# adjust/pg_cryogen

Hardware: AMD Instinct MI355X
Metric: lz4_decompress_uncompressed_GBps (higher is better)
Workload: dtype u8

## Files before the change

pg_cryogen_amd/csrc/lz4_index_pair.hip:

```cpp
#include "lz_common.h"

namespace cryo {
namespace {

constexpr uint32_t kIdxDist = 2;
constexpr uint32_t kIdxLanes = 64, kIdxRing = 512;
constexpr uint32_t kIdxLpw = 8u;
constexpr uint32_t kIdxChunk = kIdxLpw * 16u;
constexpr uint32_t kIdxWpl = kIdxLanes / kIdxLpw;
constexpr uint32_t kIdxGroups = kIdxLanes / (2u * kIdxWpl);
constexpr uint32_t kIdxLine = 16u;
constexpr uint32_t kIdxStride = kIdxRing + 16u;

constexpr uint32_t kPairTrash = kIdxLanes * kIdxStride;
constexpr uint32_t kPairPos = kPairTrash + kIdxLanes * 16u;
constexpr uint32_t kPairPosStride = (2u * kIdxLine + 8u) * 2u;
constexpr uint32_t kPairMbPos = kPairPos + kIdxLanes * kPairPosStride;
constexpr uint32_t kPairMbFilled = kPairMbPos + kIdxLanes * 4u;
constexpr uint32_t kPairLds = kPairMbFilled + kIdxLanes * 4u;
static_assert(4u * kPairLds <= 163840u, "four pairs per compute unit");

constexpr uint32_t kPairStarve = 65536u;
constexpr uint32_t kPairIdle = 65536u;

__device__ inline uint32_t pair_bperm(uint32_t v, uint32_t src_lane)
{
    return (uint32_t)__builtin_amdgcn_ds_bpermute((int)(src_lane << 2), (int)v);
}
__device__ inline uint32_t mb_load(const uint32_t *p) { return __hip_atomic_load(p, __ATOMIC_RELAXED, __HIP_MEMORY_SCOPE_WORKGROUP); }
__device__ inline void mb_store(uint32_t *p, uint32_t v) { __hip_atomic_store(p, v, __ATOMIC_RELAXED, __HIP_MEMORY_SCOPE_WORKGROUP); }

#ifndef CRYO_IDX_PAIR_WG
#define CRYO_IDX_PAIR_WG 1
#endif
#ifndef CRYO_IDX_PAIR_PRIO
#define CRYO_IDX_PAIR_PRIO 1
#endif

}

template <uint32_t PAIRS, bool PRIO>
__global__ void __launch_bounds__(128 * PAIRS)
k_lz4_idx_pair(const uint8_t *__restrict__ src_base, const uint64_t *__restrict__ src_off,
               const uint32_t *__restrict__ src_size, const uint64_t n_blocks, uint16_t *__restrict__ tbl,
               const uint32_t cap, uint2 *__restrict__ seg, uint16_t *__restrict__ dummy_base)
{
    __shared__ __attribute__((aligned(16))) uint8_t s_mem[PAIRS * kPairLds];
    const uint32_t wave = uni(threadIdx.x >> 6), lane = threadIdx.x & 63u;
    const bool feeder = wave >= PAIRS;
    const uint32_t pair = feeder ? wave - PAIRS : wave;
    uint8_t *const s_ring = s_mem + pair * kPairLds;
    uint32_t *const mb_pos = reinterpret_cast<uint32_t *>(s_ring + kPairMbPos);
    uint32_t *const mb_filled = reinterpret_cast<uint32_t *>(s_ring + kPairMbFilled);

    const uint64_t blk = ((uint64_t)blockIdx.x * PAIRS + pair) * kIdxLanes + lane;
    const bool owner = blk < n_blocks;
// ... 8 lines not shown
    const bool start_done = !owner || vend == delta;
    if (!feeder) {
        mb_pos[lane] = delta | (start_done ? 0x80000000u : 0u);
        mb_filled[lane] = 0u;
    }
    __syncthreads();

    if (feeder) {
        uint32_t requested = 0, filled = 0;
        uint32_t outA = 0, outB = 0;
        uint32_t lastp = delta;
        const uint32_t piece16 = (lane & (kIdxLpw - 1u)) * 16u;
        const uint32_t wil = lane / kIdxLpw;
#define PAIR_SRC(q) const uint64_t saoff##q = ((uint64_t)pair_bperm((uint32_t)(aoff >> 32), kIdxWpl * q + wil) << 32) | pair_bperm((uint32_t)aoff, kIdxWpl * q + wil); \
                    const uint32_t svend##q = pair_bperm(vend, kIdxWpl * q + wil);
        PAIR_SRC(0) PAIR_SRC(1) PAIR_SRC(2) PAIR_SRC(3)
        PAIR_SRC(4) PAIR_SRC(5) PAIR_SRC(6) PAIR_SRC(7)
#undef PAIR_SRC
        typedef uint32_t u32x4 __attribute__((ext_vector_type(4)));
        const uint32_t mytrash = kPairTrash + lane * 16u;
#define PAIR_SLOT(n) u32x4 fd##n = {0, 0, 0, 0}, fe##n = fd##n; uint32_t fa##n = mytrash, fb##n = fa##n;
        PAIR_SLOT(0) PAIR_SLOT(1) PAIR_SLOT(2) PAIR_SLOT(3)
        PAIR_SLOT(4) PAIR_SLOT(5) PAIR_SLOT(6) PAIR_SLOT(7)
#undef PAIR_SLOT
        uint32_t moved = 0;
        bool alldone = false;
        auto turn = [&](const uint32_t j, u32x4 &fd, u32x4 &fe, uint32_t &fa, uint32_t &fb, uint32_t &out128,
                        const uint64_t soff, const uint32_t sve, const uint64_t soff2, const uint32_t sve2) __attribute__((always_inline)) {
            const uint32_t grp = j % kIdxGroups;
            const bool myturn = lane / (2u * kIdxWpl) == grp;
            asm volatile("s_waitcnt vmcnt(%0)" ::"n"(8 * kIdxDist - 2) : "memory");
            *reinterpret_cast<u32x4 *>(s_ring + fa) = fd;
            *reinterpret_cast<u32x4 *>(s_ring + fb) = fe;
            asm volatile("" ::: "memory");
            {
                const uint32_t got = myturn ? out128 : 0u;
                filled += got;
                out128 -= got;
            }
            const uint32_t pm = mb_load(mb_pos + lane);
            const uint32_t p = pm & 0x7fffffffu;
            const bool pdone = (pm >> 31) != 0u;
            moved |= p ^ lastp;
            lastp = p;
            const bool jump = !pdone & (p >= requested) & (p < vend);
            requested = jump ? p & ~(kIdxChunk - 1u) : requested;
            filled = jump ? requested : filled;
            outA = jump ? 0u : outA;
            outB = jump ? 0u : outB;
            mb_store(mb_filled + lane, filled);
            const bool want = myturn & !pdone & (requested < vend) & (p + (kIdxRing - kIdxChunk) >= requested);
            const uint32_t wi = want ? 1u : 0u;
            const uint32_t msg = requested | wi;
            requested += wi * kIdxChunk;
            out128 |= wi * kIdxChunk;
            moved |= wi;
            const uint32_t s1 = 2u * kIdxWpl * grp + wil, s2 = s1 + kIdxWpl;
            const uint32_t m1 = pair_bperm(msg, s1), m2 = pair_bperm(msg, s2);
            const uint32_t o1 = (m1 & ~1u) + piece16, o2 = (m2 & ~1u) + piece16;
            const bool p1 = (m1 & 1u) != 0u, p2 = (m2 & 1u) != 0u;
            fa = p1 ? s1 * kIdxStride + (o1 & (kIdxRing - 1u)) : mytrash;
            fb = p2 ? s2 * kIdxStride + (o2 & (kIdxRing - 1u)) : mytrash;
            const uint8_t *g1 = src_base + (soff + ((p1 & (o1 < sve)) ? o1 : 0u));
            const uint8_t *g2 = src_base + (soff2 + ((p2 & (o2 < sve2)) ? o2 : 0u));
            asm volatile("global_load_dwordx4 %0, %1, off" : "+v"(fd) : "v"(g1));
            asm volatile("global_load_dwordx4 %0, %1, off" : "+v"(fe) : "v"(g2));
// ... 5 lines not shown
#ifdef CRYO_IDX_PROF
        const unsigned long long t_f0 = __builtin_amdgcn_s_memtime();
        uint32_t prof_rounds = 0;
#endif
        if (!wave_all(start_done)) {
            do {
                PAIR_ROUND(0, 1, 2, 3, outA)
                PAIR_ROUND(4, 5, 6, 7, outB)
#ifdef CRYO_IDX_PROF
                prof_rounds += 2u;
#endif
                idle = wave_any(moved != 0u) ? 0u : idle + 2u;
                moved = 0;
            } while (!alldone && idle < kPairIdle);
        }
#undef PAIR_ROUND
#undef PAIR_TURN
#ifdef CRYO_IDX_PROF
        if ((blockIdx.x & 255u) == 0u && lane == 0u)
            printf("[pair] feeder %u.%u: %u rounds, %llu ticks\n", blockIdx.x, pair, prof_rounds, __builtin_amdgcn_s_memtime() - t_f0);
#endif
        asm volatile("s_waitcnt vmcnt(0)" : "+v"(fd0), "+v"(fe0), "+v"(fd1), "+v"(fe1), "+v"(fd2), "+v"(fe2), "+v"(fd3), "+v"(fe3),
                                            "+v"(fd4), "+v"(fe4), "+v"(fd5), "+v"(fe5), "+v"(fd6), "+v"(fe6), "+v"(fd7), "+v"(fe7) : : "memory");
    } else {
        if (PRIO) __builtin_amdgcn_s_setprio(1);
        uint16_t *const row = tbl + blk * cap;
        uint16_t *const dummy = dummy_base + lane * 16u;
        const uint32_t kcap = cap;
        const uint32_t rb = lane * kIdxStride;
        uint32_t pos = delta, state = 0, acc = 0, tm = 0;
        uint32_t k = 0, ls = 0;
        uint32_t starved = 0;
        uint16_t *const pbuf = reinterpret_cast<uint16_t *>(s_ring + kPairPos + lane * kPairPosStride);
        uint16_t *const ptrash = pbuf + 2u * kIdxLine;
        bool done = start_done;
#ifdef CRYO_IDX_PROF
        uint32_t prof_dry = 0, prof_live = 0, prof_turns = 0;
        const unsigned long long t_w0 = __builtin_amdgcn_s_memtime();
#endif
        auto turn = [&]() __attribute__((always_inline)) {
            const uint32_t filled = mb_load(mb_filled + lane);
            asm volatile("" ::: "memory");
            const uint32_t w0 = *reinterpret_cast<const uint32_t *>(s_ring + rb + (pos & (kIdxRing - 4u)));
            const uint32_t w1 = *reinterpret_cast<const uint32_t *>(s_ring + rb + ((pos + 4u) & (kIdxRing - 4u)));
            const uint32_t w2 = *reinterpret_cast<const uint32_t *>(s_ring + rb + ((pos + 8u) & (kIdxRing - 4u)));
            const bool live = !done & (pos < vend);
            const bool canread = (pos + 8u <= filled) | (filled >= vend);
            const uint32_t x = __builtin_amdgcn_alignbyte(w1, w0, pos & 3u);
            const bool go = live & canread;
            starved = (live & !canread) ? starved + 1u : 0u;
#ifdef CRYO_IDX_PROF
            prof_dry += (live & !canread) ? 1u : 0u;
            prof_live += live ? 1u : 0u;
#endif
            const uint32_t ll = (x >> 4) & 15u, e1 = (x >> 8) & 255u, tmn = x & 15u;
            const bool l15 = ll == 15u;
            const uint32_t q2 = pos + 3u + ll + (l15 ? e1 + 1u : 0u);
            const bool tok = go & (state == 0u);
            const bool rare = tok & ((l15 & (e1 == 255u)) | (q2 > vend));
            const bool plain = tok & !rare;
            const uint32_t nx = ~x;
            const uint32_t n = nx ? (uint32_t)__builtin_ctz(nx) >> 3 : 4u;
            const bool extb = go & (state == 2u);
            *(tok ? pbuf + (k & (2u * kIdxLine - 1u)) : ptrash) = (uint16_t)(pos - delta);
            k += tok ? 1u : 0u;
            tm = tok ? tmn : tm;
            const uint32_t st_tok = tmn == 15u ? 2u : 0u;
            uint32_t npos = plain ? q2 : pos, nstate = plain ? st_tok : state;
            {
                const bool dbl = plain & !l15 & (tmn != 15u) & (ll <= 2u) & (q2 < vend) & (k < kcap);
                const uint32_t x1 = __builtin_amdgcn_alignbyte(w2, w1, pos & 3u);
                const unsigned long long xx = ((unsigned long long)x1 << 32) | x;
                const uint32_t y = (uint32_t)(xx >> (8u * (3u + ll)));
                const uint32_t llb = (y >> 4) & 15u, e1b = (y >> 8) & 255u, tmb = y & 15u;
                const bool l15b = llb == 15u;
                const uint32_t q2b = q2 + 3u + llb + (l15b ? e1b + 1u : 0u);
                const bool rec2 = dbl & !(l15b & (e1b == 255u));
                *(rec2 ? pbuf + (k & (2u * kIdxLine - 1u)) : ptrash) = (uint16_t)(q2 - delta);
                k += rec2 ? 1u : 0u;
                tm = rec2 ? tmb : tm;
                const bool last2 = rec2 & (q2b > vend);
                const bool adv2 = rec2 & !last2;
                npos = adv2 ? q2b : npos;
                nstate = adv2 ? (tmb == 15u ? 2u : 0u) : nstate;
                done = done | last2;
            }
            npos = extb ? pos + (n == 4u ? 4u : n + 1u) : npos;
            nstate = extb ? (n == 4u ? 2u : 0u) : nstate;
            done = done | !live | (k >= kcap) | (starved >= kPairStarve);
            pos = npos;
            state = nstate;
            {
                const bool longm = extb & (n == 4u) & !done;
                if (__builtin_expect(wave_any(longm), 0)) {
                    const uint32_t a0 = pos & ~3u;
                    uint32_t m = 0;
                    bool run = longm;
#pragma unroll
                    for (uint32_t kq = 0; kq < 7u; kq++) {
                        const uint32_t dq = *reinterpret_cast<const uint32_t *>(s_ring + rb + ((a0 + 4u * kq) & (kIdxRing - 4u)));
                        run = run & (dq == 0xffffffffu) & (a0 + 4u * kq + 4u <= filled);
                        m += run ? 1u : 0u;
                    }
                    const uint32_t far = a0 + 4u * m;
                    pos = (longm & (far > pos)) ? far : pos;
                }
            }
            const bool slow = rare | (!done & (state == 1u));
            if (__builtin_expect(wave_any(slow), 0)) {
                if (rare) {
                    if (l15 && e1 == 255u) { state = 1u; acc = 15u + 255u; pos += 2u; }
                    else done = true;
                } else if (slow && pos < vend && live && canread) {
                    if (n == 4u) { acc += 1020u; pos += 4u; if (acc >= vend) done = true; }
                    else {
                        acc += 255u * n + ((x >> (8u * n)) & 255u);
                        const uint32_t q = pos + n + 1u + acc;
                        if (acc >= vend || q + 2u > vend) done = true;
                        else { pos = q + 2u; state = tm == 15u ? 2u : 0u; }
                    }
                }
            }
            mb_store(mb_pos + lane, pos | (done ? 0x80000000u : 0u));
        };
#define PAIR_LINE_COPY(ps_, pd_)                                                                 \
        {                                                                                        \
            const uint4 v0_ = *reinterpret_cast<const uint4 *>(ps_);                             \
            const uint4 v1_ = *reinterpret_cast<const uint4 *>((ps_) + 8);                       \
            store16_out<false>(reinterpret_cast<uint8_t *>(pd_), v0_);                           \
            store16_out<false>(reinterpret_cast<uint8_t *>((pd_) + 8), v1_);                     \
        }
#define PAIR_PUT()                                                                               \
        {                                                                                        \
            const bool st_ = ls < k / kIdxLine;                                                  \
            const uint16_t *ps_ = pbuf + (ls & 1u) * kIdxLine;                                   \
            uint16_t *pd_ = st_ ? row + ls * kIdxLine : dummy;                                   \
            PAIR_LINE_COPY(ps_, pd_)                                                             \
            if (st_) ls++;                                                                       \
        }
        if (wave_any(!done)) {
            do {
                PAIR_PUT()
                turn(); turn(); turn(); turn();
#ifdef CRYO_IDX_PROF
                prof_turns += 4u;
#endif
            } while (wave_any(!done));
        }
#ifdef CRYO_IDX_PROF
        if ((blockIdx.x & 255u) == 0u && lane < 2u)
            printf("[pair] walker %u.%u lane %u: %u turns, live %u, dry %u, %llu ticks, k %u\n", blockIdx.x, pair, lane, prof_turns, prof_live, prof_dry,
                   __builtin_amdgcn_s_memtime() - t_w0, k);
#endif
        if (owner) {
            PAIR_PUT()
            PAIR_PUT()
            if ((k & (kIdxLine - 1u)) != 0u && ls == k / kIdxLine) {
                const uint16_t *ps_ = pbuf + (ls & 1u) * kIdxLine;
                uint16_t *pd_ = row + ls * kIdxLine;
                PAIR_LINE_COPY(ps_, pd_)
            }
            seg[blk] = make_uint2(0u, k);
        }
#undef PAIR_PUT
#undef PAIR_LINE_COPY
        if (PRIO) __builtin_amdgcn_s_setprio(0);
    }
    __syncthreads();
}

hipError_t launch_lz4_index_pair(hipStream_t s, const uint8_t *d_src, const uint64_t *d_src_off, const uint32_t *d_src_size,
                                 uint64_t n_blocks, uint32_t block_size, void *d_workspace, const Lz4IndexLayout &L)
{
    (void)block_size;
    if (n_blocks == 0) return hipSuccess;
    if (L.logS != 0u) return hipErrorInvalidValue;
    constexpr uint32_t kWg = CRYO_IDX_PAIR_WG;
    const uint64_t grid = (n_blocks + kIdxLanes * kWg - 1) / (kIdxLanes * kWg);
    if (grid > 0x7fffffffull) return hipErrorInvalidValue;
    uint8_t *ws = static_cast<uint8_t *>(d_workspace);
    hipLaunchKernelGGL((k_lz4_idx_pair<kWg, CRYO_IDX_PAIR_PRIO != 0>), dim3((uint32_t)grid), dim3(128u * kWg), 0, s, d_src, d_src_off,
                       d_src_size, n_blocks, reinterpret_cast<uint16_t *>(ws), L.cap, reinterpret_cast<uint2 *>(ws + L.seg_off),
                       reinterpret_cast<uint16_t *>(ws + L.dummy_off));
    return hipGetLastError();
}
// ... 25 lines not shown
```

pg_cryogen_amd/csrc/lz4_copy.h:

```cpp
#ifndef CRYO_LZ4_COPY_H
#define CRYO_LZ4_COPY_H

#include "lz_common.h"

namespace cryo {
namespace {

#define LDS_FENCE() asm volatile("" ::: "memory")

template <uint32_t R, uint32_t TMAX>
struct CopyLds {
    static constexpr uint32_t kBmW = TMAX / 32;
    static constexpr uint32_t kNc = TMAX / 64;
    static constexpr uint32_t kWords = kBmW + kNc;
    uint8_t *ring;
    uint8_t *in;
    uint32_t *mmeta;
    uint32_t *mbm;
};

template <uint32_t R, uint32_t SMASK>
__device__ inline void lane_runs(uint8_t *ring, const uint8_t *sbase, uint32_t rem, uint32_t sv, uint32_t dv, const bool far,
                                 const uint4 xa, const uint4 xb, uint32_t &spill)
{
    uint32_t it = 0;
    bool go = rem >= 16u;
    if (wave_any(go)) {
        do {
            const uint32_t di = dv & (R - 1u);
            if (go) {
                uint4 v = it == 0u ? xa : xb;
                if (!far) __builtin_memcpy(&v, sbase + (sv & SMASK), 16);
                __builtin_memcpy(ring + di, &v, 16);
            }
            if (go && di + 16u > R) spill = di + 16u - R;
            const uint32_t step = go ? 16u : 0u;
            sv += step; dv += step; rem -= step; it += step;
            go = rem >= 16u;
        } while (wave_any(go));
    }
    const bool lap = rem != 0u && it != 0u && !far;
    if (lap) {
        uint4 v;
        __builtin_memcpy(&v, sbase + ((sv + rem - 16u) & SMASK), 16);
        const uint32_t di = (dv + rem - 16u) & (R - 1u);
        __builtin_memcpy(ring + di, &v, 16);
        if (di + 16u > R) spill = di + 16u - R;
        rem = 0u;
    }
    if (rem != 0u) {
        uint4 v = it == 0u ? xa : xb;
        if (!far) __builtin_memcpy(&v, sbase + (sv & SMASK), 16);
        uint32_t di = dv & (R - 1u);
        if (di + rem > R) spill = di + rem - R;
        if (rem & 8u) { __builtin_memcpy(ring + di, &v.x, 8); di += 8u; v.x = v.z; v.y = v.w; }
        if (rem & 4u) { __builtin_memcpy(ring + di, &v.x, 4); di += 4u; v.x = v.y; }
        if (rem & 2u) { const uint16_t h = (uint16_t)v.x; __builtin_memcpy(ring + di, &h, 2); di += 2u; v.x >>= 16; }
        if (rem & 1u) ring[di] = (uint8_t)v.x;
    }
}


template <uint32_t R>
__device__ inline void lane_tail_pieces(uint8_t *ring, uint4 v, const uint32_t rem, uint32_t di, uint32_t &spill)
{
    if (di + rem > R) spill = di + rem - R;
    if (rem & 8u) { __builtin_memcpy(ring + di, &v.x, 8); di += 8u; v.x = v.z; v.y = v.w; }
    if (rem & 4u) { __builtin_memcpy(ring + di, &v.x, 4); di += 4u; v.x = v.y; }
    if (rem & 2u) { const uint16_t h = (uint16_t)v.x; __builtin_memcpy(ring + di, &h, 2); di += 2u; v.x >>= 16; }
    if (rem & 1u) ring[di] = (uint8_t)v.x;
}
template <uint32_t R, uint32_t N, typename T>
__device__ inline void lane_store(uint8_t *ring, const uint32_t dv, const T &v, uint32_t &spill)
{
    const uint32_t di = dv & (R - 1u);
    __builtin_memcpy(ring + di, &v, N);
    if (di + N > R) spill = di + N - R;
}

template <uint32_t R>
__device__ inline void lane_copies_v2(uint8_t *ring, const uint8_t *in, const uint32_t L, const uint32_t lpos, const uint32_t dl,
                                      const uint32_t ML, const uint32_t msrc, const uint32_t dm, const bool isfar,
                                      const uint4 xfa, const uint4 xfb, uint32_t &spill)
{
    uint4 la = make_uint4(0, 0, 0, 0), lc = la, ma = xfa;
    const bool l2 = L > 16u && L <= 32u;
    if (L != 0u) __builtin_memcpy(&la, in + (lpos & kInMask), 16);
    if (l2) __builtin_memcpy(&lc, in + ((lpos + L - 16u) & kInMask), 16);
    if (ML != 0u && !isfar) __builtin_memcpy(&ma, ring + (msrc & (R - 1u)), 16);
    if (L >= 16u) lane_store<R, 16>(ring, dl, la, spill);
    if (l2) lane_store<R, 16>(ring, dl + L - 16u, lc, spill);
    if (ML == 16u || (ML > 16u && isfar)) lane_store<R, 16>(ring, dm, ma, spill);
    if (ML >= 8u && ML < 16u) {
        const uint32_t s = ML - 8u;
        const bool hi = s >= 4u;
        const uint32_t a = hi ? ma.y : ma.x, b = hi ? ma.z : ma.y, c = hi ? ma.w : ma.z;
        const uint2 head = make_uint2(ma.x, ma.y);
        const uint2 tail = make_uint2(__builtin_amdgcn_alignbyte(b, a, s), __builtin_amdgcn_alignbyte(c, b, s));
        lane_store<R, 8>(ring, dm, head, spill);
        lane_store<R, 8>(ring, dm + s, tail, spill);
    }
    if (ML >= 4u && ML < 8u) {
        const uint32_t s = ML - 4u;
        const uint32_t tail = __builtin_amdgcn_alignbyte(ma.y, ma.x, s);
        lane_store<R, 4>(ring, dm, ma.x, spill);
        lane_store<R, 4>(ring, dm + s, tail, spill);
    }
    const bool lshort = L != 0u && L < 16u, mshort = ML != 0u && ML < 4u;
    if (wave_any(lshort | mshort)) {
        if (lshort) lane_tail_pieces<R>(ring, la, L, dl & (R - 1u), spill);
        if (mshort) lane_tail_pieces<R>(ring, ma, ML, dm & (R - 1u), spill);
    }
    if (wave_any(L > 32u)) {
        const uint4 z = make_uint4(0, 0, 0, 0);
        lane_runs<R, kInMask>(ring, in, L > 32u ? L - 16u : 0u, lpos + 16u, dl + 16u, false, z, z, spill);
    }
    if (wave_any(ML > 16u)) {
        const uint32_t done = isfar ? 16u : 0u;
        lane_runs<R, R - 1u>(ring, ring, ML > 16u ? ML - done : 0u, msrc + done, dm + done, isfar, xfb, xfb, spill);
    }
}

template <uint32_t R, uint32_t TMAX, bool NOLIT = false>
__device__ inline void seq_copy(Wave<R> &w, const CopyLds<R, TMAX> &L, const uint32_t nseq, const uint32_t ostart,
                                const uint32_t ll, const uint32_t ml, const uint32_t off, const uint32_t lpos,
                                const uint32_t T, const bool isfar, const uint4 xfa, const uint4 xfb, Stats &st)
{
    static_assert(R - TMAX >= TMAX + 1023u, "an offset must be either in the ring or flushed");
    constexpr uint32_t kBmW = CopyLds<R, TMAX>::kBmW, kNc = CopyLds<R, TMAX>::kNc;
    const uint32_t lane = w.lane;
    const uint32_t op0 = w.op;
    const bool act = lane < nseq;
    st.batches++;
    st.batch_seqs += nseq;

    const uint32_t mrel = ostart + ll;
    const bool indep = act && (isfar || off >= mrel + ml);
    const bool dep = act && !indep;
    const uint32_t mlx = dep ? ml : 0u;
    const uint32_t mend = scan64_incl(mlx);
    const uint32_t mcum = mend - mlx;
    const uint32_t MT = lane_get(mend, 63u);
    const unsigned long long depm = wave_ballot(dep);
    const uint32_t drank = __builtin_amdgcn_mbcnt_hi((uint32_t)(depm >> 32), __builtin_amdgcn_mbcnt_lo((uint32_t)depm, 0u));

    {
    if (lane < kBmW) L.mbm[lane] = 0u;
    LDS_FENCE();
    if (dep) {
        static_assert(TMAX < 2048u, "11 bits");
        L.mmeta[drank] = (mrel - mcum) | (off << 11);
        if (mcum != 0u) atomicOr(&L.mbm[(mcum - 1u) >> 5], 1u << ((mcum - 1u) & 31u));
    }
    LDS_FENCE();
// ... 94 lines not shown
```

pg_cryogen_amd/csrc/lz4_dec2.hip:

```cpp
#include "lz_common.h"
#include "lz4_copy.h"
#include <cstdio>
#include <cstdlib>

namespace cryo {


constexpr uint32_t kSeqWin = 1536;
constexpr uint32_t kT2 = 1536;

template <bool MULTI>
struct IndexRow {
    const uint16_t *base;
    uint2 sd;
    uint32_t cap_s, ext, npieces, pc;
    const uint16_t *t0, *t1, *t2;
    uint32_t len0, len1, len2, n0;

    __device__ inline void find(const uint16_t *&t, uint32_t &len)
    {
        len = 0;
        t = base;
        while (pc < npieces) {
            const uint32_t sg = pc >> 1;
            const uint32_t dx = lane_get(sd.x, sg), dy = lane_get(sd.y, sg);
            const uint32_t l = (pc & 1u) ? dy : (dx & 0xffffu);
            const uint32_t b = sg * cap_s + ((pc & 1u) ? ext + (dx >> 16) : 0u);
            pc++;
            if (l != 0u) { t = base + b; len = l; break; }
        }
    }
    __device__ inline void open(const uint16_t *row, const uint2 *seg, const uint64_t blk, const uint32_t logS, const uint32_t cap_s_,
                                const uint32_t ext_, const uint32_t lane)
    {
        base = row;
        cap_s = cap_s_; ext = ext_;
        npieces = 2u << logS;
        sd = make_uint2(0, 0);
        if (lane < (1u << logS)) sd = seg[(blk << logS) + lane];
        pc = 0; n0 = 0;
        find(t0, len0);
        t1 = t2 = base; len1 = len2 = 0;
        if (MULTI) { find(t1, len1); find(t2, len2); }
    }
    __device__ inline uint32_t avail(const uint32_t k) const
    {
        const uint32_t have = MULTI ? len0 + len1 + len2 : len0, at = n0 + k;
        return at < have ? (have - at < 64u ? have - at : 64u) : 0u;
    }
    __device__ inline uint32_t entry(const uint32_t k, const uint32_t lane) const
    {
        const uint32_t i = n0 + k + lane;
        uint32_t e = 0;
        if (MULTI) {
            const uint16_t *q = i < len0 ? t0 + i : (i < len0 + len1 ? t1 + (i - len0) : t2 + (i - len0 - len1));
            if (i < len0 + len1 + len2) e = *q;
        } else if (i < len0) e = t0[i];
        return e;
    }
    __device__ inline void advance(const uint32_t n)
    {
        n0 += n;
        while (MULTI && len0 != 0u && n0 >= len0) {
            n0 -= len0;
            t0 = t1; len0 = len1;
            t1 = t2; len1 = len2;
            find(t2, len2);
        }
    }
};

__device__ inline uint32_t lane_next(uint32_t v)
{
    return (uint32_t)__builtin_amdgcn_update_dpp(0, (int)v, 0x130 , 0xf, 0xf, false);
}

template <uint32_t R, bool MULTI>
__device__ inline uint32_t lz4_seq_batch(Wave<R> &w, const CopyLds<R, kT2> &L, uint32_t &vp, const uint32_t B,
                                         const uint32_t epos, const uint32_t navail, const IndexRow<MULTI> &ix, uint32_t &epre, Stats &st,
                                         unsigned long long *stop_hist = nullptr)
{
    const uint32_t lane = w.lane;
    const uint32_t vend = w.vend;
    if (vend < 32u || B < 32u || navail == 0u) return 0;
    const uint32_t vsafe = vend - 16u;
    if (vp + 64u > vsafe || w.op + 64u > B) return 0;
    stamp(st, 7);
    while (w.in_hi < vend && w.in_hi < vp + kSeqWin) w.refill_deferred();
    LDS_FENCE();
    uint2 mir = make_uint2(0, 0);
    if (lane < 2u) mir = *reinterpret_cast<const uint2 *>(L.in + lane * 8u);
    else if (lane < 4u) mir = *reinterpret_cast<const uint2 *>(L.ring + (lane - 2u) * 8u);
    stamp(st, 0);
    const uint32_t pos = vp + ((epos + w.delta - vp) & 0xffffu);
    const bool cand = lane < navail && pos + 8u <= vp + kSeqWin;
    const uint32_t rp = cand ? pos : vp;
    const uint32_t t = L.in[rp & kInMask];
    const uint32_t e1 = L.in[(rp + 1u) & kInMask];
    uint32_t ll = t >> 4;
    uint32_t k = 1u;
    if (ll == 15u) { ll += e1; k = 2u; }
    const uint32_t q = rp + k + ll;
    const bool inwin = q + 8u <= vp + kSeqWin;
    const uint32_t rq = inwin ? q : vp;
    const uint32_t off = (uint32_t)L.in[rq & kInMask] | ((uint32_t)L.in[(rq + 1u) & kInMask] << 8);
    const uint32_t e2 = L.in[(rq + 2u) & kInMask];
    if (lane < 2u) *reinterpret_cast<uint2 *>(L.in + kInRing + lane * 8u) = mir;
    else if (lane < 4u) *reinterpret_cast<uint2 *>(L.ring + R + (lane - 2u) * 8u) = mir;
    uint32_t ml = (t & 15u) + 4u;
    uint32_t dlen = k + ll + 2u;
    const bool hasM = (t & 15u) == 15u;
    if (hasM) { ml += e2; dlen += 1u; }
    const uint32_t outlen = cand ? ll + ml : 0u;
    const uint32_t oend = scan64_incl(outlen);
    const uint32_t ostart = oend - outlen;
    const uint32_t mabs = w.op + ostart + ll;
    const uint32_t npos = lane_next(pos);
    const bool chain = (lane == 0u ? pos == vp : true) && (lane + 1u >= navail || lane == 63u || npos == pos + dlen);
    constexpr uint32_t kNear = R - kT2;
    constexpr uint32_t kOvlMax = 64;
    const bool isfar = cand && off >= kNear;
    const bool ok = cand && inwin && chain && !(t >= 0xf0u && e1 == 255u) && !(hasM && e2 == 255u) && (off >= ml || (off != 0u && ml <= kOvlMax)) && off <= mabs &&
                    pos + dlen <= vsafe && oend <= kT2 && w.op + oend + 16u <= B && !(isfar && ml > 32u);
    const unsigned long long badmask = wave_ballot(!ok);
    const uint32_t nseq = badmask ? ctz64(badmask) : 64u;
    if (st.on && stop_hist && badmask && nseq < navail && lane == nseq) {
        const int why = !cand ? 0 : !inwin ? 1 : !chain ? 2 : (t >= 0xf0u && e1 == 255u) ? 3 : (hasM && e2 == 255u) ? 4 : (off < ml && (off == 0u || ml > kOvlMax)) ? 5 : off > mabs ? 6
                        : pos + dlen > vsafe ? 7 : oend > kT2 ? 8 : w.op + oend + 16u > B ? 9 : 10;
        atomicAdd(&stop_hist[why], 1ull);
    }
    stamp(st, 1);
    if (!(st.ablate & 2u)) w.flush();
    else w.flushed = w.op & ~(kChunk - 1u);
    stamp(st, 2);
    if (!(st.ablate & 4u)) w.top_up(); else w.nstale = 0;
    if (nseq == 0u) return 0;
    const uint32_t T = lane_get(oend, nseq - 1u);
    const uint32_t used = lane_get(pos + dlen, nseq - 1u) - vp;
    epre = ix.entry(nseq, lane);
    uint4 xfa, xfb;
    asm volatile("" : "=v"(xfa.x), "=v"(xfa.y), "=v"(xfa.z), "=v"(xfa.w), "=v"(xfb.x), "=v"(xfb.y), "=v"(xfb.z), "=v"(xfb.w));
    if (lane < nseq && isfar && !(st.ablate & 1u)) {
        const uint8_t *g = w.dst + (mabs - off);
        __builtin_memcpy(&xfa, g, 16);
        __builtin_memcpy(&xfb, g + 16, 16);
    }
    stamp(st, 3);
    seq_copy<R, kT2>(w, L, nseq, ostart, ll, ml, off, pos + k, T, isfar, xfa, xfb, st);
    vp += used;
    stamp(st, 0);
    return nseq;
}

template <uint32_t R>
__device__ inline uint32_t lz4_general_seq(Wave<R> &w, uint32_t &vp, const uint32_t B)
{
    const uint32_t lane = w.lane, vend = w.vend;
    w.flush();
    w.need(vp);
    uint32_t win = w.window(vp);

    const uint32_t token = lane_get(win, 0);
    uint32_t ll = token >> 4;
    uint32_t k = 1;
    if (ll == 15u) {
        uint32_t wbase = vp;
        for (;;) {
            const unsigned long long m = wave_ballot(win != 255u) & ~((1ull << k) - 1ull);
            if (m != 0ull) {
                const uint32_t f = ctz64(m);
                ll += (f - k) * 255u + lane_get(win, f);
                k = f + 1u;
                break;
            }
            if (wbase + 63u + 16u >= vend) return 2u;
            ll += (64u - k) * 255u;
            wbase += 64u;
            w.need(wbase);
            win = w.window(wbase);
// ... 113 lines not shown
    bool done = bad;
    uint32_t skip = 0;
    IndexRow<MULTI> ix;
    ix.open(tbl + uni64(blk * (uint64_t)tbl_cap), seg, blk, logS, cap_s, ext, lane);
    uint32_t poor = 0;

    uint32_t efirst = 0;
    if (!bad) efirst = ix.entry(0, lane);
    bool have_first = !bad;
    if (!bad) {
        w.prefetch();
        w.refill();
        if (w.in_hi < w.vend) w.refill();
    }
    uint32_t npre = ix.avail(0);

    while (!done) {
        if (skip == 0u) {
            uint32_t n;
            uint32_t epre = efirst;
            bool have_pre = have_first;
            bool more;
            have_first = false;
            do {
                uint32_t e = epre, navail = npre;
                if (!have_pre) { navail = ix.avail(0); e = ix.entry(0, lane); }
                n = lz4_seq_batch<R, MULTI>(w, L, vp, B, e, navail, ix, epre, st, STATS ? stats + 16 : nullptr);
                have_pre = n != 0u;
                npre = ix.avail(n);
                ix.advance(n);
                if (n == 0u) st.zero_batches++;
                more = n >= 8u || (n != 0u && n == navail);
            } while (more);
            poor = n < 4u ? poor + 1u : 0u;
            if (poor >= 3u) { skip = 8u; poor = 0u; }
        } else {
            skip--;
        }
        st.general_seqs++;
        ix.advance(1u);
        const uint32_t r = lz4_general_seq<R>(w, vp, B);
        if (r == 2u) { bad = true; break; }
        if (r == 1u) done = true;
    }

    if (!bad && w.op != B) bad = true;
    if (!bad) {
        w.flush();
        w.flush_tail();
    }
    if (lane == 0) status[blk] = bad ? CRYO_ST_CORRUPT : CRYO_ST_OK;
    if (STATS && lane == 0) {
        atomicAdd(&stats[0], (unsigned long long)st.batches);
        atomicAdd(&stats[1], (unsigned long long)st.batch_seqs);
        atomicAdd(&stats[2], (unsigned long long)st.general_seqs);
        atomicAdd(&stats[3], (unsigned long long)st.chunks);
        atomicAdd(&stats[4], (unsigned long long)st.rounds);
        atomicAdd(&stats[5], (unsigned long long)st.zero_batches);
        stamp(st, 7);
        for (int k = 0; k < 8; k++) atomicAdd(&stats[8 + k], st.t[k]);
    }
}

#ifndef CRYO_DUAL_PROF
#define CRYO_DUAL_PROF 0
#endif
// ... 341 lines not shown
```

pg_cryogen_amd/csrc/lz_common.h:

```cpp
#ifndef CRYO_LZ_COMMON_H
#define CRYO_LZ_COMMON_H


#include "kernels.h"

namespace cryo {
namespace {


constexpr uint32_t kInRing = 2048, kInMask = kInRing - 1;
constexpr uint32_t kChunk = 1024;
constexpr uint32_t kInChunk = 512;

__device__ inline uint32_t uni(uint32_t v) { return __builtin_amdgcn_readfirstlane(v); }
__device__ inline unsigned long long wave_ballot(bool p) { return __builtin_amdgcn_ballot_w64(p); }
__device__ inline bool wave_any(bool p) { return __builtin_amdgcn_ballot_w64(p) != 0ull; }
__device__ inline bool wave_all(bool p) { return __builtin_amdgcn_ballot_w64(!p) == 0ull; }
__device__ inline uint64_t uni64(uint64_t v)
{
    const uint32_t lo = __builtin_amdgcn_readfirstlane((uint32_t)v);
    const uint32_t hi = __builtin_amdgcn_readfirstlane((uint32_t)(v >> 32));
    return ((uint64_t)hi << 32) | lo;
}
__device__ inline uint32_t lane_get(uint32_t v, uint32_t l) { return __builtin_amdgcn_readlane(v, l); }
// ... 83 lines not shown
        if (o < vend) v = *reinterpret_cast<const uint2 *>(abase + o);
        return v;
    }
    __device__ inline void prefetch()
    {
        pre = fetch(in_hi);
        pre2 = fetch(in_hi + kInChunk);
        pre3 = fetch(in_hi + 2u * kInChunk);
        nstale = 0;
    }
    __device__ inline void refill()
    {
        *reinterpret_cast<uint2 *>(in + ((in_hi + lane * 8u) & kInMask)) = pre;
        in_hi += kInChunk;
        pre = pre2;
        pre2 = pre3;
        pre3 = fetch(in_hi + 2u * kInChunk);
    }
    __device__ inline void refill_deferred()
    {
        *reinterpret_cast<uint2 *>(in + ((in_hi + lane * 8u) & kInMask)) = pre;
        in_hi += kInChunk;
        pre = pre2;
        pre2 = pre3;
        nstale++;
    }
    __device__ inline void top_up()
    {
        if (nstale >= 3u) pre = fetch(in_hi);
        if (nstale >= 2u) pre2 = fetch(in_hi + kInChunk);
        if (nstale >= 1u) pre3 = fetch(in_hi + 2u * kInChunk);
        nstale = 0;
    }
    __device__ inline void need(uint32_t vp)
    {
        while (in_hi < vend && vp + 128u > in_hi) refill();
    }
    __device__ inline uint32_t window(uint32_t vp) const { return in[(vp + lane) & kInMask]; }

    __device__ inline void flush()
    {
        while (op - flushed >= kChunk) {
            if (dst_aligned) {
                const uint4 x = *reinterpret_cast<const uint4 *>(ring + ((flushed + lane * 16u) & (R - 1)));
                store16_out<CRYO_NT_FLUSH != 0>(dst + flushed + lane * 16u, x);
            } else {
                for (uint32_t i = lane; i < kChunk; i += 64u) dst[flushed + i] = ring[(flushed + i) & (R - 1)];
            }
            flushed += kChunk;
        }
    }
    __device__ inline void flush_tail()
    {
        for (uint32_t i = flushed + lane; i < op; i += 64u) dst[i] = ring[i & (R - 1)];
        flushed = op;
    }
};

template <int CTRL, int ROW_MASK>
__device__ inline uint32_t dpp_add(uint32_t x)
{
    return x + (uint32_t)__builtin_amdgcn_update_dpp(0, (int)x, CTRL, ROW_MASK, 0xf, false);
}
__device__ inline uint32_t scan16_incl(uint32_t x)
{
    x = dpp_add<0x111, 0xf>(x);
// ... 224 lines not shown
```

Before: 1139.

## Walk up to three LZ4 tokens per turn with a mirrored ring tail

The index walker now parses up to three consecutive LZ4 sequence tokens per turn, replacing the previous limit of two. The parsing moves into a shared host/device helper that uses byte-perm lookups over a 16-byte window. The feeder also mirrors the first 16 bytes of each ring into a tail region, so the walker can read five contiguous words without wrap masking. Records are written unconditionally to pbuf, with k advanced only by the count of valid records, which removes the trash-pointer selects. The aim is fewer serial turns per token, paid for with extra LDS stores in the feeder and more ALU work per turn.

New measurement: 1147, median of 6. About the same (+0.7%).

```diff
diff --git a/pg_cryogen_amd/csrc/lz4_hop.h b/pg_cryogen_amd/csrc/lz4_hop.h
--- /dev/null
+++ b/pg_cryogen_amd/csrc/lz4_hop.h
@@ -0,0 +1,126 @@
+#ifndef CRYO_LZ4_HOP_H
+#define CRYO_LZ4_HOP_H
+
+#include <stdint.h>
+
+#if defined(__HIPCC__)
+#define LZ4_HOP_FN __host__ __device__ inline
+#else
+#define LZ4_HOP_FN inline
+#endif
+
+constexpr uint32_t kLz4HopWindow = 16u;
+constexpr uint32_t kLz4HopTokens = 3u;
+constexpr uint32_t kLz4HopFirst = 8u;
+constexpr uint32_t kLz4HopLast = 13u;
+
+struct Lz4Hop {
+    uint32_t nrec;
+    uint32_t rec1;
+    uint32_t rec2;
+    uint32_t adv;
+    uint32_t state;
+    uint32_t tm;
+    uint32_t n;
+    bool done;
+    bool rare;
+    bool went;
+};
+
+LZ4_HOP_FN uint32_t lz4_hop_perm(const uint32_t hi, const uint32_t lo, const uint32_t sel)
+{
+#if defined(__HIP_DEVICE_COMPILE__)
+    return __builtin_amdgcn_perm(hi, lo, sel);
+#else
+    const uint64_t v = ((uint64_t)hi << 32) | lo;
+    uint32_t r = 0;
+    for (uint32_t i = 0; i < 4u; i++) {
+        const uint32_t c = (sel >> (8u * i)) & 255u;
+        r |= (c < 8u ? (uint32_t)(v >> (8u * c)) & 255u : 0u) << (8u * i);
+    }
+    return r;
+#endif
+}
+
+LZ4_HOP_FN uint32_t lz4_hop_align(const uint32_t hi, const uint32_t lo, const uint32_t s)
+{
+#if defined(__HIP_DEVICE_COMPILE__)
+    return __builtin_amdgcn_alignbyte(hi, lo, s);
+#else
+    return (uint32_t)((((uint64_t)hi << 32) | lo) >> (8u * s));
+#endif
+}
+
+LZ4_HOP_FN uint32_t lz4_hop_at(const uint32_t w0, const uint32_t w1, const uint32_t u0, const uint32_t u1, const uint32_t o)
+{
+    const uint32_t sel = o * 0x0101u + 0x0100u;
+    const uint32_t a = lz4_hop_perm(w1, w0, sel), b = lz4_hop_perm(u1, u0, sel - 0x0707u);
+    return o >= 7u ? b : a;
+}
+
+LZ4_HOP_FN Lz4Hop lz4_hop(const uint32_t w0, const uint32_t w1, const uint32_t w2, const uint32_t w3, const uint32_t valid,
+                          const uint32_t dist, const uint32_t room, const uint32_t state)
+{
+    Lz4Hop h;
+    const bool go = (dist != 0u) & (valid >= kLz4HopFirst);
+    const bool tok = go & (state == 0u);
+    const bool extb = go & (state == 2u);
+    const uint32_t nx = ~w0;
+    h.n = nx ? (uint32_t)__builtin_ctz(nx) >> 3 : 4u;
+    h.went = go;
+    const uint32_t reach = valid - 1u < kLz4HopLast + 1u ? valid - 1u : kLz4HopLast + 1u;
+    const uint32_t lat = reach < dist ? reach : dist;
+    const uint32_t u0 = lz4_hop_align(w2, w1, 3u), u1 = lz4_hop_align(w3, w2, 3u);
+    const uint32_t ll = (w0 >> 4) & 15u, e1 = (w0 >> 8) & 255u, tmn = w0 & 15u;
+    const bool l15 = ll == 15u;
+    const uint32_t q1 = 3u + ll + (l15 ? e1 + 1u : 0u);
+    h.rare = tok & ((l15 & (e1 == 255u)) | (q1 > dist));
+    const bool plain = tok & !h.rare;
+    const bool t1 = plain & (tmn != 15u) & (q1 < lat);
+    const uint32_t y = lz4_hop_at(w0, w1, u0, u1, q1);
+    const uint32_t llb = (y >> 4) & 15u, e1b = (y >> 8) & 255u, tmb = y & 15u;
+    const bool l15b = llb == 15u;
+    const uint32_t q2 = q1 + 3u + llb + (l15b ? e1b + 1u : 0u);
+    const bool r1 = t1 & !(l15b & (e1b == 255u));
+    const bool last1 = r1 & (q2 > dist);
+    const bool a1 = r1 & !last1;
+    const bool t2 = a1 & (tmb != 15u) & (q2 < lat);
+    const uint32_t z = lz4_hop_at(w0, w1, u0, u1, q2);
+    const uint32_t llc = (z >> 4) & 15u, e1c = (z >> 8) & 255u, tmc = z & 15u;
+    const bool l15c = llc == 15u;
+    const uint32_t q3 = q2 + 3u + llc + (l15c ? e1c + 1u : 0u);
+    const bool r2 = t2 & !(l15c & (e1c == 255u));
+    const bool last2 = r2 & (q3 > dist);
+    const bool a2 = r2 & !last2;
+    const uint32_t nrec = r2 ? 3u : r1 ? 2u : tok ? 1u : 0u;
+    h.nrec = nrec < room ? nrec : room;
+    h.rec1 = q1;
+    h.rec2 = q2;
+    h.tm = tmn;
+    h.done = last1 | last2;
+    const uint32_t nib = a2 ? tmc : a1 ? tmb : tmn;
+    h.adv = a2 ? q3 : a1 ? q2 : plain ? q1 : extb ? (h.n == 4u ? 4u : h.n + 1u) : 0u;
+    h.state = plain ? (nib == 15u ? 2u : 0u) : extb ? (h.n == 4u ? 2u : 0u) : state;
+    return h;
+}
+
+LZ4_HOP_FN bool lz4_hop_rare(const Lz4Hop &h, const uint32_t w0, const uint32_t vend, uint32_t &pos, uint32_t &state,
+                             uint32_t &acc, uint32_t &tm)
+{
+    if (h.rare) {
+        const uint32_t ll = (w0 >> 4) & 15u, e1 = (w0 >> 8) & 255u;
+        if (ll == 15u && e1 == 255u) { state = 1u; acc = 15u + 255u; tm = h.tm; pos += 2u; return false; }
+        return true;
+    }
+    if (state == 1u && pos < vend && h.went) {
+        if (h.n == 4u) { acc += 1020u; pos += 4u; return acc >= vend; }
+        acc += 255u * h.n + ((w0 >> (8u * h.n)) & 255u);
+        const uint32_t q = pos + h.n + 1u + acc;
+        if (acc >= vend || q + 2u > vend) return true;
+        pos = q + 2u;
+        state = tm == 15u ? 2u : 0u;
+    }
+    return false;
+}
+
+#endif
diff --git a/pg_cryogen_amd/csrc/lz4_index_pair.hip b/pg_cryogen_amd/csrc/lz4_index_pair.hip
--- a/pg_cryogen_amd/csrc/lz4_index_pair.hip
+++ b/pg_cryogen_amd/csrc/lz4_index_pair.hip
@@ -1,4 +1,5 @@
 #include "lz_common.h"
+#include "lz4_hop.h"
 
 namespace cryo {
 namespace {
@@ -22,6 +23,7 @@
 
 constexpr uint32_t kPairStarve = 65536u;
 constexpr uint32_t kPairIdle = 65536u;
+constexpr uint32_t kPairDone = 0x80000000u;
 
 __device__ inline uint32_t pair_bperm(uint32_t v, uint32_t src_lane)
 {
@@ -96,6 +98,11 @@
             asm volatile("s_waitcnt vmcnt(%0)" ::"n"(8 * kIdxDist - 2) : "memory");
             *reinterpret_cast<u32x4 *>(s_ring + fa) = fd;
             *reinterpret_cast<u32x4 *>(s_ring + fb) = fe;
+            {
+                const uint32_t r1 = (2u * kIdxWpl * grp + wil) * kIdxStride, r2 = r1 + kIdxWpl * kIdxStride;
+                *reinterpret_cast<u32x4 *>(s_ring + (fa == r1 ? r1 + kIdxRing : mytrash)) = fd;
+                *reinterpret_cast<u32x4 *>(s_ring + (fb == r2 ? r2 + kIdxRing : mytrash)) = fe;
+            }
             asm volatile("" ::: "memory");
             {
                 const uint32_t got = myturn ? out128 : 0u;
@@ -167,67 +174,42 @@
         uint32_t k = 0, ls = 0;
         uint32_t starved = 0;
         uint16_t *const pbuf = reinterpret_cast<uint16_t *>(s_ring + kPairPos + lane * kPairPosStride);
-        uint16_t *const ptrash = pbuf + 2u * kIdxLine;
-        bool done = start_done;
-#ifdef CRYO_IDX_PROF
-        uint32_t prof_dry = 0, prof_live = 0, prof_turns = 0;
+        uint32_t dn = start_done ? kPairDone : 0u;
+#ifdef CRYO_IDX_PROF
+        uint32_t prof_dry = 0, prof_live = 0, prof_turns = 0, prof_tok = 0;
         const unsigned long long t_w0 = __builtin_amdgcn_s_memtime();
 #endif
         auto turn = [&]() __attribute__((always_inline)) {
             const uint32_t filled = mb_load(mb_filled + lane);
             asm volatile("" ::: "memory");
-            const uint32_t w0 = *reinterpret_cast<const uint32_t *>(s_ring + rb + (pos & (kIdxRing - 4u)));
-            const uint32_t w1 = *reinterpret_cast<const uint32_t *>(s_ring + rb + ((pos + 4u) & (kIdxRing - 4u)));
-            const uint32_t w2 = *reinterpret_cast<const uint32_t *>(s_ring + rb + ((pos + 8u) & (kIdxRing - 4u)));
-            const bool live = !done & (pos < vend);
-            const bool canread = (pos + 8u <= filled) | (filled >= vend);
-            const uint32_t x = __builtin_amdgcn_alignbyte(w1, w0, pos & 3u);
-            const bool go = live & canread;
-            starved = (live & !canread) ? starved + 1u : 0u;
-#ifdef CRYO_IDX_PROF
-            prof_dry += (live & !canread) ? 1u : 0u;
+            const uint32_t sh = pos & 3u;
+            const uint32_t *const rd = reinterpret_cast<const uint32_t *>(s_ring + rb + (pos & (kIdxRing - 4u)));
+            const uint32_t d0 = rd[0], d1 = rd[1], d2 = rd[2], d3 = rd[3], d4 = rd[4];
+            static_assert(kIdxRing - 4u + 20u <= kIdxStride && kLz4HopWindow <= kIdxStride - kIdxRing, "the window ends inside the mirror");
+            const uint32_t w0 = lz4_hop_align(d1, d0, sh), w1 = lz4_hop_align(d2, d1, sh);
+            const uint32_t w2 = lz4_hop_align(d3, d2, sh), w3 = lz4_hop_align(d4, d3, sh);
+            const bool live = (dn == 0u) & (pos < vend);
+            const int have = (int)(filled - pos);
+            const uint32_t valid = filled >= vend ? kLz4HopWindow : (uint32_t)(have < 0 ? 0 : have > (int)kLz4HopWindow ? (int)kLz4HopWindow : have);
+            const Lz4Hop h = lz4_hop(w0, w1, w2, w3, valid, live ? vend - pos : 0u, kcap - k, state);
+            starved = (live & !h.went) ? starved + 1u : 0u;
+#ifdef CRYO_IDX_PROF
+            prof_dry += (live & !h.went) ? 1u : 0u;
             prof_live += live ? 1u : 0u;
-#endif
-            const uint32_t ll = (x >> 4) & 15u, e1 = (x >> 8) & 255u, tmn = x & 15u;
-            const bool l15 = ll == 15u;
-            const uint32_t q2 = pos + 3u + ll + (l15 ? e1 + 1u : 0u);
-            const bool tok = go & (state == 0u);
-            const bool rare = tok & ((l15 & (e1 == 255u)) | (q2 > vend));
-            const bool plain = tok & !rare;
-            const uint32_t nx = ~x;
-            const uint32_t n = nx ? (uint32_t)__builtin_ctz(nx) >> 3 : 4u;
-            const bool extb = go & (state == 2u);
-            *(tok ? pbuf + (k & (2u * kIdxLine - 1u)) : ptrash) = (uint16_t)(pos - delta);
-            k += tok ? 1u : 0u;
-            tm = tok ? tmn : tm;
-            const uint32_t st_tok = tmn == 15u ? 2u : 0u;
-            uint32_t npos = plain ? q2 : pos, nstate = plain ? st_tok : state;
-            {
-                const bool dbl = plain & !l15 & (tmn != 15u) & (ll <= 2u) & (q2 < vend) & (k < kcap);
-                const uint32_t x1 = __builtin_amdgcn_alignbyte(w2, w1, pos & 3u);
-                const unsigned long long xx = ((unsigned long long)x1 << 32) | x;
-                const uint32_t y = (uint32_t)(xx >> (8u * (3u + ll)));
-                const uint32_t llb = (y >> 4) & 15u, e1b = (y >> 8) & 255u, tmb = y & 15u;
-                const bool l15b = llb == 15u;
-                const uint32_t q2b = q2 + 3u + llb + (l15b ? e1b + 1u : 0u);
-                const bool rec2 = dbl & !(l15b & (e1b == 255u));
-                *(rec2 ? pbuf + (k & (2u * kIdxLine - 1u)) : ptrash) = (uint16_t)(q2 - delta);
-                k += rec2 ? 1u : 0u;
-                tm = rec2 ? tmb : tm;
-                const bool last2 = rec2 & (q2b > vend);
-                const bool adv2 = rec2 & !last2;
-                npos = adv2 ? q2b : npos;
-                nstate = adv2 ? (tmb == 15u ? 2u : 0u) : nstate;
-                done = done | last2;
-            }
-            npos = extb ? pos + (n == 4u ? 4u : n + 1u) : npos;
-            nstate = extb ? (n == 4u ? 2u : 0u) : nstate;
-            done = done | !live | (k >= kcap) | (starved >= kPairStarve);
-            pos = npos;
-            state = nstate;
-            {
-                const bool longm = extb & (n == 4u) & !done;
-                if (__builtin_expect(wave_any(longm), 0)) {
+            prof_tok += h.nrec;
+#endif
+            const uint32_t base = pos - delta;
+            pbuf[k & (2u * kIdxLine - 1u)] = (uint16_t)base;
+            pbuf[(k + 1u) & (2u * kIdxLine - 1u)] = (uint16_t)(base + h.rec1);
+            pbuf[(k + 2u) & (2u * kIdxLine - 1u)] = (uint16_t)(base + h.rec2);
+            k += h.nrec;
+            dn = (h.done | !live | (k >= kcap) | (starved >= kPairStarve)) ? kPairDone : dn;
+            const bool ext4 = h.went & (state == 2u) & (h.n == 4u);
+            pos += h.adv;
+            state = h.state;
+            if (__builtin_expect(wave_any(ext4 | h.rare | (state == 1u)), 0)) {
+                const bool longm = ext4 & (dn == 0u);
+                if (wave_any(longm)) {
                     const uint32_t a0 = pos & ~3u;
                     uint32_t m = 0;
                     bool run = longm;
@@ -240,24 +222,13 @@
                     const uint32_t far = a0 + 4u * m;
                     pos = (longm & (far > pos)) ? far : pos;
                 }
+                const bool slow = h.rare | ((dn == 0u) & (state == 1u));
+                if (slow && lz4_hop_rare(h, w0, vend, pos, state, acc, tm)) dn = kPairDone;
+                state = dn != 0u ? 0u : state;
             }
-            const bool slow = rare | (!done & (state == 1u));
-            if (__builtin_expect(wave_any(slow), 0)) {
-                if (rare) {
-                    if (l15 && e1 == 255u) { state = 1u; acc = 15u + 255u; pos += 2u; }
-                    else done = true;
-                } else if (slow && pos < vend && live && canread) {
-                    if (n == 4u) { acc += 1020u; pos += 4u; if (acc >= vend) done = true; }
-                    else {
-                        acc += 255u * n + ((x >> (8u * n)) & 255u);
-                        const uint32_t q = pos + n + 1u + acc;
-                        if (acc >= vend || q + 2u > vend) done = true;
-                        else { pos = q + 2u; state = tm == 15u ? 2u : 0u; }
-                    }
-                }
-            }
-            mb_store(mb_pos + lane, pos | (done ? 0x80000000u : 0u));
+            mb_store(mb_pos + lane, pos | dn);
         };
+        static_assert(4u * kLz4HopTokens <= kIdxLine && kIdxLine - 1u + 4u * kLz4HopTokens < 2u * kIdxLine, "pbuf holds four turns behind a PAIR_PUT");
 #define PAIR_LINE_COPY(ps_, pd_)                                                                 \
         {                                                                                        \
             const uint4 v0_ = *reinterpret_cast<const uint4 *>(ps_);                             \
@@ -273,19 +244,19 @@
             PAIR_LINE_COPY(ps_, pd_)                                                             \
             if (st_) ls++;                                                                       \
         }
-        if (wave_any(!done)) {
+        if (wave_any(dn == 0u)) {
             do {
                 PAIR_PUT()
                 turn(); turn(); turn(); turn();
 #ifdef CRYO_IDX_PROF
                 prof_turns += 4u;
 #endif
-            } while (wave_any(!done));
+            } while (wave_any(dn == 0u));
         }
 #ifdef CRYO_IDX_PROF
         if ((blockIdx.x & 255u) == 0u && lane < 2u)
-            printf("[pair] walker %u.%u lane %u: %u turns, live %u, dry %u, %llu ticks, k %u\n", blockIdx.x, pair, lane, prof_turns, prof_live, prof_dry,
-                   __builtin_amdgcn_s_memtime() - t_w0, k);
+            printf("[pair] walker %u.%u lane %u: %u turns, live %u, dry %u, %llu ticks, k %u, tokens %u\n", blockIdx.x, pair, lane, prof_turns, prof_live,
+                   prof_dry, __builtin_amdgcn_s_memtime() - t_w0, k, prof_tok);
 #endif
         if (owner) {
             PAIR_PUT()
```

## Issue input prefetch loads unconditionally and defer their consumption across batches

Applied to the files above, without the earlier changes.

Replaces the conditional top_up with top_up_all, which always issues three clamped global loads into staging registers and commits them later in take_up at the start of the next batch. The top-up is also moved after the far-match loads so those loads are in flight together. The goal is to hide global load latency behind the sequence copy instead of waiting on it inside the batch. Alongside this, lane_runs now handles a 16-byte tail directly, the unused lane_copies_v2 helpers are deleted, and the single-table index entry lookup is clamped rather than branched. The cost is more registers, redundant loads when nothing is stale, and extra complexity in the ordering between refill and take_up.

Measured after the change: 1137 before, 1148 after (median of 6 runs). About the same (+0.9%).

```diff
diff --git a/pg_cryogen_amd/csrc/lz4_copy.h b/pg_cryogen_amd/csrc/lz4_copy.h
--- a/pg_cryogen_amd/csrc/lz4_copy.h
+++ b/pg_cryogen_amd/csrc/lz4_copy.h
@@ -24,7 +24,7 @@
                                  const uint4 xa, const uint4 xb, uint32_t &spill)
 {
     uint32_t it = 0;
-    bool go = rem >= 16u;
+    bool go = rem > 16u;
     if (wave_any(go)) {
         do {
             const uint32_t di = dv & (R - 1u);
@@ -36,7 +36,7 @@
             if (go && di + 16u > R) spill = di + 16u - R;
             const uint32_t step = go ? 16u : 0u;
             sv += step; dv += step; rem -= step; it += step;
-            go = rem >= 16u;
+            go = rem > 16u;
         } while (wave_any(go));
     }
     const bool lap = rem != 0u && it != 0u && !far;
@@ -53,6 +53,7 @@
         if (!far) __builtin_memcpy(&v, sbase + (sv & SMASK), 16);
         uint32_t di = dv & (R - 1u);
         if (di + rem > R) spill = di + rem - R;
+        if (rem & 16u) __builtin_memcpy(ring + di, &v, 16);
         if (rem & 8u) { __builtin_memcpy(ring + di, &v.x, 8); di += 8u; v.x = v.z; v.y = v.w; }
         if (rem & 4u) { __builtin_memcpy(ring + di, &v.x, 4); di += 4u; v.x = v.y; }
         if (rem & 2u) { const uint16_t h = (uint16_t)v.x; __builtin_memcpy(ring + di, &h, 2); di += 2u; v.x >>= 16; }
@@ -60,66 +61,6 @@
     }
 }
 
-
-template <uint32_t R>
-__device__ inline void lane_tail_pieces(uint8_t *ring, uint4 v, const uint32_t rem, uint32_t di, uint32_t &spill)
-{
-    if (di + rem > R) spill = di + rem - R;
-    if (rem & 8u) { __builtin_memcpy(ring + di, &v.x, 8); di += 8u; v.x = v.z; v.y = v.w; }
-    if (rem & 4u) { __builtin_memcpy(ring + di, &v.x, 4); di += 4u; v.x = v.y; }
-    if (rem & 2u) { const uint16_t h = (uint16_t)v.x; __builtin_memcpy(ring + di, &h, 2); di += 2u; v.x >>= 16; }
-    if (rem & 1u) ring[di] = (uint8_t)v.x;
-}
-template <uint32_t R, uint32_t N, typename T>
-__device__ inline void lane_store(uint8_t *ring, const uint32_t dv, const T &v, uint32_t &spill)
-{
-    const uint32_t di = dv & (R - 1u);
-    __builtin_memcpy(ring + di, &v, N);
-    if (di + N > R) spill = di + N - R;
-}
-
-template <uint32_t R>
-__device__ inline void lane_copies_v2(uint8_t *ring, const uint8_t *in, const uint32_t L, const uint32_t lpos, const uint32_t dl,
-                                      const uint32_t ML, const uint32_t msrc, const uint32_t dm, const bool isfar,
-                                      const uint4 xfa, const uint4 xfb, uint32_t &spill)
-{
-    uint4 la = make_uint4(0, 0, 0, 0), lc = la, ma = xfa;
-    const bool l2 = L > 16u && L <= 32u;
-    if (L != 0u) __builtin_memcpy(&la, in + (lpos & kInMask), 16);
-    if (l2) __builtin_memcpy(&lc, in + ((lpos + L - 16u) & kInMask), 16);
-    if (ML != 0u && !isfar) __builtin_memcpy(&ma, ring + (msrc & (R - 1u)), 16);
-    if (L >= 16u) lane_store<R, 16>(ring, dl, la, spill);
-    if (l2) lane_store<R, 16>(ring, dl + L - 16u, lc, spill);
-    if (ML == 16u || (ML > 16u && isfar)) lane_store<R, 16>(ring, dm, ma, spill);
-    if (ML >= 8u && ML < 16u) {
-        const uint32_t s = ML - 8u;
-        const bool hi = s >= 4u;
-        const uint32_t a = hi ? ma.y : ma.x, b = hi ? ma.z : ma.y, c = hi ? ma.w : ma.z;
-        const uint2 head = make_uint2(ma.x, ma.y);
-        const uint2 tail = make_uint2(__builtin_amdgcn_alignbyte(b, a, s), __builtin_amdgcn_alignbyte(c, b, s));
-        lane_store<R, 8>(ring, dm, head, spill);
-        lane_store<R, 8>(ring, dm + s, tail, spill);
-    }
-    if (ML >= 4u && ML < 8u) {
-        const uint32_t s = ML - 4u;
-        const uint32_t tail = __builtin_amdgcn_alignbyte(ma.y, ma.x, s);
-        lane_store<R, 4>(ring, dm, ma.x, spill);
-        lane_store<R, 4>(ring, dm + s, tail, spill);
-    }
-    const bool lshort = L != 0u && L < 16u, mshort = ML != 0u && ML < 4u;
-    if (wave_any(lshort | mshort)) {
-        if (lshort) lane_tail_pieces<R>(ring, la, L, dl & (R - 1u), spill);
-        if (mshort) lane_tail_pieces<R>(ring, ma, ML, dm & (R - 1u), spill);
-    }
-    if (wave_any(L > 32u)) {
-        const uint4 z = make_uint4(0, 0, 0, 0);
-        lane_runs<R, kInMask>(ring, in, L > 32u ? L - 16u : 0u, lpos + 16u, dl + 16u, false, z, z, spill);
-    }
-    if (wave_any(ML > 16u)) {
-        const uint32_t done = isfar ? 16u : 0u;
-        lane_runs<R, R - 1u>(ring, ring, ML > 16u ? ML - done : 0u, msrc + done, dm + done, isfar, xfb, xfb, spill);
-    }
-}
 
 template <uint32_t R, uint32_t TMAX, bool NOLIT = false>
 __device__ inline void seq_copy(Wave<R> &w, const CopyLds<R, TMAX> &L, const uint32_t nseq, const uint32_t ostart,
diff --git a/pg_cryogen_amd/csrc/lz4_dec2.hip b/pg_cryogen_amd/csrc/lz4_dec2.hip
--- a/pg_cryogen_amd/csrc/lz4_dec2.hip
+++ b/pg_cryogen_amd/csrc/lz4_dec2.hip
@@ -55,7 +55,10 @@
         if (MULTI) {
             const uint16_t *q = i < len0 ? t0 + i : (i < len0 + len1 ? t1 + (i - len0) : t2 + (i - len0 - len1));
             if (i < len0 + len1 + len2) e = *q;
-        } else if (i < len0) e = t0[i];
+        } else {
+            const uint32_t last = len0 != 0u ? len0 - 1u : 0u;
+            e = t0[i < last ? i : last];
+        }
         return e;
     }
     __device__ inline void advance(const uint32_t n)
@@ -82,6 +85,7 @@
 {
     const uint32_t lane = w.lane;
     const uint32_t vend = w.vend;
+    w.take_up();
     if (vend < 32u || B < 32u || navail == 0u) return 0;
     const uint32_t vsafe = vend - 16u;
     if (vp + 64u > vsafe || w.op + 64u > B) return 0;
@@ -133,11 +137,6 @@
     if (!(st.ablate & 2u)) w.flush();
     else w.flushed = w.op & ~(kChunk - 1u);
     stamp(st, 2);
-    if (!(st.ablate & 4u)) w.top_up(); else w.nstale = 0;
-    if (nseq == 0u) return 0;
-    const uint32_t T = lane_get(oend, nseq - 1u);
-    const uint32_t used = lane_get(pos + dlen, nseq - 1u) - vp;
-    epre = ix.entry(nseq, lane);
     uint4 xfa, xfb;
     asm volatile("" : "=v"(xfa.x), "=v"(xfa.y), "=v"(xfa.z), "=v"(xfa.w), "=v"(xfb.x), "=v"(xfb.y), "=v"(xfb.z), "=v"(xfb.w));
     if (lane < nseq && isfar && !(st.ablate & 1u)) {
@@ -145,6 +144,11 @@
         __builtin_memcpy(&xfa, g, 16);
         __builtin_memcpy(&xfb, g + 16, 16);
     }
+    if (!(st.ablate & 4u)) w.top_up_all(); else w.nstale = 0;
+    if (nseq == 0u) return 0;
+    const uint32_t T = lane_get(oend, nseq - 1u);
+    const uint32_t used = lane_get(pos + dlen, nseq - 1u) - vp;
+    epre = ix.entry(nseq, lane);
     stamp(st, 3);
     seq_copy<R, kT2>(w, L, nseq, ostart, ll, ml, off, pos + k, T, isfar, xfa, xfb, st);
     vp += used;
@@ -324,6 +328,7 @@
                 if (n == 0u) st.zero_batches++;
                 more = n >= 8u || (n != 0u && n == navail);
             } while (more);
+            w.take_up();
             poor = n < 4u ? poor + 1u : 0u;
             if (poor >= 3u) { skip = 8u; poor = 0u; }
         } else {
diff --git a/pg_cryogen_amd/csrc/lz_common.h b/pg_cryogen_amd/csrc/lz_common.h
--- a/pg_cryogen_amd/csrc/lz_common.h
+++ b/pg_cryogen_amd/csrc/lz_common.h
@@ -139,6 +139,26 @@
         if (nstale >= 1u) pre3 = fetch(in_hi + 2u * kInChunk);
         nstale = 0;
     }
+    uint2 nw = {0, 0}, nw2 = {0, 0}, nw3 = {0, 0};
+    uint32_t npend = 0;
+    __device__ inline void top_up_all()
+    {
+        const uint32_t o = in_hi + lane * 8u, last = (vend - 1u) & ~7u;
+        const uint32_t l1 = nstale >= 3u ? last : 0u, l2 = nstale >= 2u ? last : 0u, l3 = nstale >= 1u ? last : 0u;
+        const uint32_t o2 = o + kInChunk, o3 = o + 2u * kInChunk;
+        nw = *reinterpret_cast<const uint2 *>(abase + (o < l1 ? o : l1));
+        nw2 = *reinterpret_cast<const uint2 *>(abase + (o2 < l2 ? o2 : l2));
+        nw3 = *reinterpret_cast<const uint2 *>(abase + (o3 < l3 ? o3 : l3));
+        npend = nstale;
+        nstale = 0;
+    }
+    __device__ inline void take_up()
+    {
+        if (npend >= 3u) pre = nw;
+        if (npend >= 2u) pre2 = nw2;
+        if (npend >= 1u) pre3 = nw3;
+        npend = 0;
+    }
     __device__ inline void need(uint32_t vp)
     {
         while (in_hi < vend && vp + 128u > in_hi) refill();
```
